# sijieaaa/AGPlace

Measured on AMD Instinct MI355X. Metric: aerial-ground pairs/sec (backbone+ODE+pool), higher is better.
Workload: dtype f16 (fp16 x fp16, fp32 accumulate); 1 GPU; nuScenes-AG 6-cam (C3/C4): MM.forward_q on [b,3,224,1344] + DBVanilla2D on [b,1,3,224,224], ResNet18 stem+layer1-3, euler h=0.1 x3 FCODE, GeM, stage-2 fusion; inference forward; the voxel branch's pooled outputs enter as fixed tensors (SURVEY.md 8d); global_batch=64, parallelism=dp1, bn=per-rank (eval: running statistics), paired_trunks=True, hipgraph=True, steps_in_flight=2, library_default_precision=4, headline_is_library_default=True, streams=2, query_sub_batches_on_streams=1, query_input=fp32 normalised panorama

## Files before the change

### agplace_amd/csrc/fblock64.hip

```cpp

#include <type_traits>
#include <utility>

#include "igemm_params.hpp"

namespace agp_fb {

constexpr int MAXP = 4;
constexpr int TW = 28;
constexpr int RING = 16;
constexpr int ROWB = 32 * 128;
constexpr int TAB_OFF = 2 * RING * ROWB + 512;
constexpr int STRIP_OFF = TAB_OFF + 4 * 64 * 4;
template <bool POOL> constexpr int lds_bytes() { return STRIP_OFF + 4 * 2048; }

struct Problem {
    const void* x; void* out;
    const void* w1; const void* w2;
    const float *s1, *t1, *s2, *t2;
    float* pool;
    uint32_t bytes;
    int VR, HP, W, pitch;
    int nstrips, segs;
    int dbg;
    FastDiv d_hp, d_segs;
};
struct Group {
    Problem p[MAXP];
    int wg_end[MAXP];
    int nprob;
};

__device__ __forceinline__ int perm23(int r) { return (r & 0x13) | ((r & 4) << 1) | ((r & 8) >> 1); }

template <bool POOL, bool M16, class... RF>
__global__ void __launch_bounds__(512, 2) fblock64_kernel(Group g, RF... rf) {
#if defined(__HIP_DEVICE_COMPILE__)
    constexpr bool RG = sizeof...(RF) != 0;
    extern __shared__ __attribute__((aligned(16))) char smem[];
    char* const XR = smem;
    char* const IR = smem + RING * ROWB;
    float* const tab = (float*)(smem + TAB_OFF);

    const int tid = threadIdx.x, lane = tid & 63;
    const int wave = __builtin_amdgcn_readfirstlane(tid >> 6);
    const int role = wave >> 2, cA = wave & 1, pA = (wave >> 1) & 1;
    const int l31 = lane & 31, lh = lane >> 5;
    const int la = lane & 15, kq = lane >> 4;

    const int bid = blockIdx.x;
    int pid = 0, lb = bid;
    {
        const int e0 = g.wg_end[0], e1 = g.wg_end[1], e2 = g.wg_end[2], np = g.nprob;
        if (np > 1 && bid >= e0) { pid = 1; lb = bid - e0; }
        if (np > 2 && bid >= e1) { pid = 2; lb = bid - e1; }
        if (np > 3 && bid >= e2) { pid = 3; lb = bid - e2; }
    }
    const Problem& p = g.p[pid];
    const int VR = p.VR, HP = p.HP, W = p.W, pitch = p.pitch, segs = p.segs;
    const FastDiv d_hp = p.d_hp;
    const int dbg = p.dbg;
    const int strip = (int)fdiv((uint32_t)lb, p.d_segs);
    const int sk = lb - strip * segs;
    const int Ra = (int)(((uint32_t)sk * (uint32_t)VR / (uint32_t)segs) & ~1u);
    const int Rb = sk + 1 == segs ? VR : (int)(((uint32_t)(sk + 1) * (uint32_t)VR / (uint32_t)segs) & ~1u);
    const int x0 = strip * TW;
    const int NS = (Rb - Ra + 3) >> 2;

    f16x8 w[36];
    {
        const bf16_t* wb = (const bf16_t*)(role ? p.w2 : p.w1);
        int i = 0;
        if constexpr (!M16) {
            const bf16_t* wp = wb + (size_t)(cA * 32 + perm23(l31)) * 576 + lh * 8;
#pragma unroll
            for (int ky = 0; ky < 3; ++ky)
#pragma unroll
                for (int cc = 0; cc < 2; ++cc)
#pragma unroll
                    for (int kx = 0; kx < 3; ++kx)
#pragma unroll
                        for (int ks = 0; ks < 2; ++ks, ++i)
                            w[i] = *(const f16x8*)(wp + (ky * 3 + kx) * 64 + cc * 32 + ks * 16);
        } else {
#pragma unroll
            for (int ky = 0; ky < 3; ++ky)
#pragma unroll
                for (int cc = 0; cc < 2; ++cc)
#pragma unroll
                    for (int kx = 0; kx < 3; ++kx)
#pragma unroll
                        for (int ct = 0; ct < 2; ++ct, ++i)
                            w[i] = *(const f16x8*)(wb + (size_t)(cA * 32 + 8 * (la >> 2) + 4 * ct + (la & 3)) * 576 + (ky * 3 + kx) * 64 + cc * 32 + kq * 8);
        }
    }
    if (tid < 64) {
        tab[tid] = p.s1[tid];
        tab[64 + tid] = p.t1[tid];
        tab[128 + tid] = p.s2[tid];
        tab[192 + tid] = p.t2[tid];
    }

    int A[3];
#pragma unroll
    for (int kx = 0; kx < 3; ++kx) {
        const int s = (M16 ? la : l31) + kx;
        A[kx] = s * 128 + (((M16 ? kq : lh) ^ ((s >> 1) & 7)) << 4);
    }
    const int px0 = M16 ? la : l31, px1 = M16 ? la + 16 : l31;
    const int ch0 = M16 ? kq : lh, ch1 = M16 ? kq : lh + 2;
    auto slot_off = [&](int s, int c) { return s * 128 + (((4 * cA + c) ^ ((s >> 1) & 7)) << 4); };
    const int wr0 = slot_off(px0, ch0), wr1 = slot_off(px1, ch1);
    const int rr0 = slot_off(px0 + 2, ch0), rr1 = slot_off(px1 + 2, ch1);
    const float* const tb0 = tab + role * 128 + 32 * cA + 8 * ch0;
    const float* const tb1 = tab + role * 128 + 32 * cA + 8 * ch1;
    const bool cin0 = (x0 - 1 + px0 >= 0) && (x0 - 1 + px0 < W), cin1 = (x0 - 1 + px1 >= 0) && (x0 - 1 + px1 < W);
    const bool ctk0 = cin0 && px0 < TW + 2, ctk1 = cin1 && px1 < TW + 2;
    const bool sok0 = px0 < TW && x0 + px0 < W, sok1 = px1 < TW && x0 + px1 < W;
    char* const ostrip = smem + STRIP_OFF + (wave & 3) * 2048;
    auto strip_off = [&](int px, int c) { return px * 64 + ((c ^ ((px >> 1) & 3)) << 4); };
    const int sw0 = strip_off(px0, ch0), sw1 = strip_off(px1, ch1);
    const int spx = lane >> 2;
    const int sr_ = strip_off(spx, lane & 3);
    const int gline = (x0 + 1 + spx) * 128 + 64 * cA + 16 * (lane & 3);
    const bool st_ok0 = spx < TW && x0 + spx < W, st_ok1 = spx + 16 < TW && x0 + spx + 16 < W;

    const __amdgpu_buffer_rsrc_t rx = __builtin_amdgcn_make_buffer_rsrc((void*)p.x, 0, p.bytes, 0x00020000);
    const int pc = wave & 3;
    int dvoff;
    {
        const int s = pc * 8 + (lane >> 3);
        int xp = x0 - 1 + s;
        xp = xp < 0 ? 0 : (xp > W + 1 ? W + 1 : xp);
        dvoff = xp * 128 + (((lane & 7) ^ ((s >> 1) & 7)) << 4);
    }
    auto issue_rows = [&](int R0, int cnt) {
#pragma unroll 4
        for (int r = 0; r < cnt; ++r) {
            const int R = R0 + r;
            const int Rc = R < 0 ? 0 : (R >= VR ? VR - 1 : R);
            const int so = __builtin_amdgcn_readfirstlane(Rc * pitch);
            __builtin_amdgcn_raw_ptr_buffer_load_lds(rx, LDS_PTR(XR + (R & (RING - 1)) * ROWB + pc * 1024), 16, dvoff, so, 0, 0);
        }
    };
    auto is_real = [&](int R) -> bool {
        if (R < 0 || R >= VR) return false;
        const int yy = R - (int)fdiv((uint32_t)R, d_hp) * HP;
        return yy >= 1 && yy <= HP - 2;
    };
    struct Acc {
        f32x16 m;
        f32x4 t[2][2];
    };
    auto acc_zero = [](Acc& a) {
        if constexpr (!M16) {
#pragma unroll
            for (int r = 0; r < 16; ++r) a.m[r] = 0.f;
        } else {
#pragma unroll
            for (int i = 0; i < 2; ++i)
#pragma unroll
                for (int j = 0; j < 2; ++j) a.t[i][j] = f32x4{0.f, 0.f, 0.f, 0.f};
        }
    };
    auto tile2 = [&](const char* ring, int R, Acc& a0, Acc& a1, auto&& mid, auto&& epi0) {
        acc_zero(a0);
        acc_zero(a1);
        constexpr int NG = M16 ? 24 : 48, PD = 2, NF = M16 ? 2 : 1;
        const char* rb[4];
#pragma unroll
        for (int q = 0; q < 4; ++q) rb[q] = ring + __builtin_amdgcn_readfirstlane(((R - 1 + q) & (RING - 1)) * ROWB);
        f16x8 fb[PD + 1][NF];
        auto load_group = [&](auto gc, auto slotc) {
            constexpr int g = decltype(gc)::value, sl = decltype(slotc)::value;
            if constexpr (M16) {
                constexpr int q = g / 6, cc = (g % 6) / 3, kx = g % 3;
                fb[sl][0] = *(const f16x8*)(rb[q] + (A[kx] ^ (cc << 6)));
                fb[sl][1] = *(const f16x8*)(rb[q] + (A[kx] ^ (cc << 6)) + 2048);
            } else {
                constexpr int q = g / 12, cc = (g % 12) / 6, kx = (g % 6) / 2, ks = g % 2;
                fb[sl][0] = *(const f16x8*)(rb[q] + (A[kx] ^ ((cc * 4 + ks * 2) << 4)));
            }
        };
        auto do_group = [&](auto gc, auto slotc) {
            constexpr int g = decltype(gc)::value, sl = decltype(slotc)::value;
            if constexpr (M16) {
                constexpr int q = g / 6, j = (g % 6) * 2;
#pragma unroll
                for (int ct = 0; ct < 2; ++ct) {
                    if constexpr (q <= 2) {
                        a0.t[ct][0] = __builtin_amdgcn_mfma_f32_16x16x32_f16(w[q * 12 + j + ct], fb[sl][0], a0.t[ct][0], 0, 0, 0);
                        a0.t[ct][1] = __builtin_amdgcn_mfma_f32_16x16x32_f16(w[q * 12 + j + ct], fb[sl][1], a0.t[ct][1], 0, 0, 0);
                    }
                    if constexpr (q >= 1) {
                        a1.t[ct][0] = __builtin_amdgcn_mfma_f32_16x16x32_f16(w[(q - 1) * 12 + j + ct], fb[sl][0], a1.t[ct][0], 0, 0, 0);
                        a1.t[ct][1] = __builtin_amdgcn_mfma_f32_16x16x32_f16(w[(q - 1) * 12 + j + ct], fb[sl][1], a1.t[ct][1], 0, 0, 0);
                    }
                }
            } else {
                constexpr int q = g / 12, j = g % 12;
                if constexpr (q <= 2) a0.m = __builtin_amdgcn_mfma_f32_32x32x16_f16(w[q * 12 + j], fb[sl][0], a0.m, 0, 0, 0);
                if constexpr (q >= 1) a1.m = __builtin_amdgcn_mfma_f32_32x32x16_f16(w[(q - 1) * 12 + j], fb[sl][0], a1.m, 0, 0, 0);
            }
        };
        auto step = [&](auto gc, auto&& self) -> void {
            constexpr int g = decltype(gc)::value;
            if constexpr (g < NG) {
                if constexpr (g + PD < NG) load_group(std::integral_constant<int, g + PD>{}, std::integral_constant<int, (g + PD) % (PD + 1)>{});
                __builtin_amdgcn_sched_barrier(0);
                do_group(gc, std::integral_constant<int, g % (PD + 1)>{});
                __builtin_amdgcn_sched_barrier(0);
                if constexpr (g == (M16 ? 4 : 8)) mid();
                if constexpr (g == 3 * NG / 4 - 1) epi0();
                self(std::integral_constant<int, g + 1>{}, self);
            }
        };
        load_group(std::integral_constant<int, 0>{}, std::integral_constant<int, 0>{});
        load_group(std::integral_constant<int, 1>{}, std::integral_constant<int, 1>{});
        if constexpr (PD > 2) load_group(std::integral_constant<int, 2>{}, std::integral_constant<int, 2>{});
        step(std::integral_constant<int, 0>{}, step);
    };
    auto bn = [&](const Acc& a, float* v) {
#pragma unroll
        for (int u = 0; u < 2; ++u) {
            const float* tb = u ? tb1 : tb0;
            const f32x4 s0 = *(const f32x4*)(tb), s1 = *(const f32x4*)(tb + 4);
            const f32x4 t0 = *(const f32x4*)(tb + 64), t1 = *(const f32x4*)(tb + 64 + 4);
#pragma unroll
            for (int e = 0; e < 4; ++e) {
                const float c0 = M16 ? a.t[0][u][e] : a.m[8 * u + e], c1 = M16 ? a.t[1][u][e] : a.m[8 * u + 4 + e];
                v[8 * u + e] = c0 * s0[e] + t0[e];
                v[8 * u + 4 + e] = c1 * s1[e] + t1[e];
            }
        }
    };
    RangeTrack<RG> rg;
    auto track16 = [&](const float* v, bool ok0, bool ok1) {
        RangeTrack<RG> t0, t1;
#pragma unroll
        for (int e = 0; e < 8; e += 2) { t0.pos2(v[e], v[e + 1]); t1.pos2(v[8 + e], v[9 + e]); }
        rg.pos2(ok0 ? t0.hi : 0.f, ok1 ? t1.hi : 0.f);
    };
    auto write_ir = [&](int R, const Acc& acc, bool real) {
        char* const dst = IR + __builtin_amdgcn_readfirstlane((R & (RING - 1)) * ROWB);
        float v[16];
        bn(acc, v);
        if constexpr (RG) track16(v, real && ctk0, real && ctk1);
        u32x4 o0 = pack8_h_lo(v, 0.f), o1 = pack8_h_lo(v + 8, 0.f);
        if (!(real && cin0)) o0 = u32x4{0u, 0u, 0u, 0u};
        if (!(real && cin1)) o1 = u32x4{0u, 0u, 0u, 0u};
        *(u32x4*)(dst + wr0) = o0;
        *(u32x4*)(dst + wr1) = o1;
    };
    auto conv1_pair = [&](int R) {
        const bool real0 = is_real(R), real1 = is_real(R + 1);
        Acc a0, a1;
        if (real0 || real1) {
            tile2(XR, R, a0, a1, [] {}, [&] { write_ir(R, a0, real0); });
            write_ir(R + 1, a1, real1);
        } else {
            acc_zero(a0);
            write_ir(R, a0, false);
            write_ir(R + 1, a0, false);
        }
    };
    f32x4 pacc[2];
    const __amdgpu_buffer_rsrc_t ro = __builtin_amdgcn_make_buffer_rsrc(p.out, 0, p.bytes, 0x00020000);
    u32x4 pl0 = {0u, 0u, 0u, 0u}, pl1 = {0u, 0u, 0u, 0u};
    int poff = -1;
    const int gl0 = st_ok0 ? gline : -(1 << 30), gl1 = st_ok1 ? gline + 2048 : -(1 << 30);
    auto store_lines = [&](const u32x4& l0, const u32x4& l1, int off) {
        const int v0 = (off >= 0 && gl0 >= 0) ? off + gl0 : -16, v1 = (off >= 0 && gl1 >= 0) ? off + gl1 : -16;
        if (!(dbg & 1)) {
            __builtin_amdgcn_raw_buffer_store_b128(l0, ro, v0, 0, 0);
            __builtin_amdgcn_raw_buffer_store_b128(l1, ro, v1, 0, 0);
        }
    };
    auto flush_pending = [&]() { store_lines(pl0, pl1, poff); poff = -1; };
    auto epi2 = [&](int R, const Acc& acc, bool real, u32x4& l0, u32x4& l1, bool first) {
        const char* const rsrc = XR + __builtin_amdgcn_readfirstlane((R & (RING - 1)) * ROWB);
        u32x4 r0 = {0u, 0u, 0u, 0u}, r1 = r0;
        if (!(dbg & 16)) { r0 = *(const u32x4*)(rsrc + rr0); r1 = *(const u32x4*)(rsrc + rr1); }
        float v[16], rf[16];
        bn(acc, v);
        unpack8_h(r0, rf);
        unpack8_h(r1, rf + 8);
#pragma unroll
        for (int e = 0; e < 16; ++e) v[e] += rf[e];
        if constexpr (RG) track16(v, real && sok0, real && sok1);
        u32x4 o0 = pack8_h_lo(v, 0.f), o1 = pack8_h_lo(v + 8, 0.f);
        if constexpr (POOL) {
            if (!sok0) o0 = u32x4{0u, 0u, 0u, 0u};
            if (!sok1) o1 = u32x4{0u, 0u, 0u, 0u};
        }
        *(u32x4*)(ostrip + sw0) = o0;
        *(u32x4*)(ostrip + sw1) = o1;
        l0 = *(const u32x4*)(ostrip + sr_);
        l1 = *(const u32x4*)(ostrip + sr_ + 1024);
        if constexpr (POOL) {
            if (first) { pacc[0] = f32x4{0.f, 0.f, 0.f, 0.f}; pacc[1] = pacc[0]; }
            {
                const int tpx = 8 * (lane >> 4) + ((lane >> 2) & 3), pp = lane & 3;
                const int tr0 = tpx * 64 + (((pp >> 1) ^ ((tpx >> 1) & 3)) << 4) + 8 * (pp & 1);
                typedef __attribute__((ext_vector_type(4))) short s16x4;
                const uint32_t one2 = real ? 0x3C003C00u : 0u;
                const f16x8 ones = __builtin_bit_cast(f16x8, u32x4{one2, one2, one2, one2});
#pragma unroll
                for (int ct = 0; ct < 2; ++ct) {
                    const s16x4 b0 = __builtin_amdgcn_ds_read_tr16_b64_v4i16((__attribute__((address_space(3))) s16x4*)(ostrip + (tr0 ^ (32 * ct))));
                    const s16x4 b1 = __builtin_amdgcn_ds_read_tr16_b64_v4i16((__attribute__((address_space(3))) s16x4*)(ostrip + (((tr0 + 256) ^ 32) ^ (32 * ct))));
                    const bf16x8 bf = __builtin_shufflevector(b0, b1, 0, 1, 2, 3, 4, 5, 6, 7);
                    pacc[ct] = __builtin_amdgcn_mfma_f32_16x16x32_f16(ones, __builtin_bit_cast(f16x8, bf), pacc[ct], 0, 0, 0);
                }
            }
        }
    };
    auto conv2_pair = [&](int R) {
        const bool real0 = is_real(R), real1 = is_real(R + 1);
        if (!(real0 || real1)) {
            if constexpr (POOL) { pacc[0] = f32x4{0.f, 0.f, 0.f, 0.f}; pacc[1] = pacc[0]; }
            return;
        }
        Acc a0, a1;
        u32x4 q0, q1;
        tile2(IR, R, a0, a1, flush_pending, [&] { epi2(R, a0, real0, q0, q1, true); });
        epi2(R + 1, a1, real1, pl0, pl1, false);
        store_lines(q0, q1, real0 ? __builtin_amdgcn_readfirstlane(R * pitch) : -1);
        poff = real1 ? __builtin_amdgcn_readfirstlane((R + 1) * pitch) : -1;
    };
    auto pool_flush = [&](int R) {
        if constexpr (POOL) {
            if (p.pool != nullptr && lane < 16) {
                float* o = p.pool + ((size_t)(R >> 1) * p.nstrips + strip) * 64 + 32 * cA + lane;
                o[0] = pacc[0][0];
                o[16] = pacc[1][0];
            }
        }
    };

    if (role == 0) issue_rows(Ra - 2, 8);
    __builtin_amdgcn_s_waitcnt(0x0070);
    __builtin_amdgcn_s_barrier();
    if (role == 0 && pA == 0) conv1_pair(Ra - 1);
    asm volatile("s_waitcnt lgkmcnt(0)" ::: "memory");
    __builtin_amdgcn_s_barrier();
    for (int t = 0; t <= NS; ++t) {
        if (role == 0) {
            if (t < NS) {
                if (t + 1 < NS && !(dbg & 2)) issue_rows(Ra + 4 * t + 6, 4);
                const int R = Ra + 1 + 4 * t + 2 * pA;
                if (R <= Rb) conv1_pair(R);
            }
            asm volatile("s_waitcnt vmcnt(0)" ::: "memory");
        } else if (t >= 1) {
            const int R = Ra + 4 * (t - 1) + 2 * pA;
            if (R < Rb) {
                conv2_pair(R);
                pool_flush(R);
            }
        }
        asm volatile("s_waitcnt lgkmcnt(0)" ::: "memory");
        if (!(dbg & 4)) __builtin_amdgcn_s_barrier();
    }
    if (role == 1) flush_pending();
    rg.flush(rg_word(rf...), 0.f);
#endif
}

}

using namespace agp_fb;

static int fb_num_cus() {
    static int n = -1;
    if (n < 0) {
        int dev = 0, v = 0;
        if (hipGetDevice(&dev) != hipSuccess || hipDeviceGetAttribute(&v, hipDeviceAttributeMultiprocessorCount, dev) != hipSuccess || v <= 0) v = 256;
        n = v;
    }
    return n;
}

static bool fb_desc_ok(const agp_bblock64_desc* d) {
    return d && d->in && d->out && d->w1 && d->w2 && d->scale1 && d->shift1 && d->scale2 && d->shift2 && d->n > 0 && d->h > 0 && d->w > 0 &&
           (d->h & 1) == 0 && (int64_t)d->n * (d->h + 2) * (d->w + 2) * 128 < (1ll << 31);
}

extern "C" int64_t agp_bblock64_pool_floats(const agp_bblock64_desc* d) {
    if (!fb_desc_ok(d)) return 0;
    return (int64_t)d->n * ((d->h + 2) / 2) * ((d->w + TW - 1) / TW) * 64;
}

extern "C" int agp_bblock64_fwd_grouped(const agp_bblock64_desc* descs, int n, void* stream) {
    if (!descs || n < 1 || n > MAXP) return AGP_E_BADARG;
    Group g = {};
    g.nprob = n;
    bool pool = false;
    int64_t total = 0;
    for (int i = 0; i < n; ++i) {
        const agp_bblock64_desc* d = descs + i;
        if (!fb_desc_ok(d)) return AGP_E_BADARG;
        Problem& p = g.p[i];
        p.x = d->in; p.out = d->out; p.w1 = d->w1; p.w2 = d->w2;
        p.s1 = d->scale1; p.t1 = d->shift1; p.s2 = d->scale2; p.t2 = d->shift2;
        p.pool = d->pool_partial;
        pool = pool || d->pool_partial;
        p.HP = d->h + 2; p.VR = d->n * p.HP; p.W = d->w; p.pitch = (d->w + 2) * 128;
        p.bytes = (uint32_t)((int64_t)p.VR * p.pitch);
        p.nstrips = (d->w + TW - 1) / TW;
        p.d_hp = make_fastdiv((uint32_t)p.HP);
        p.dbg = AGP_TUNE("FB_DBG", 0);
        total += (int64_t)p.nstrips * p.VR;
    }
    const int cus = fb_num_cus();
    int wg = 0;
    for (int i = 0; i < n; ++i) {
        Problem& p = g.p[i];
        int64_t s = (int64_t)p.VR * cus / total;
        const int64_t smax = p.VR / 16 > 1 ? p.VR / 16 : 1;
        s = s < 1 ? 1 : (s > smax ? smax : s);
        while (s > 1 && s * (int64_t)p.VR >= (1ll << 32)) --s;
        p.segs = (int)s;
        p.d_segs = make_fastdiv((uint32_t)p.segs);
        wg += p.nstrips * p.segs;
        g.wg_end[i] = wg;
    }
    const int form = descs[0].form == 0 ? 1 : 0;
    static std::atomic<uint64_t> attr_done[2][2][2];
    uint32_t* const rflag = agp_range_flag_get();
    auto launch = [&](auto... rf) {
        constexpr bool RG = sizeof...(rf) != 0;
        const void* fn = pool ? (form ? (const void*)fblock64_kernel<true, true, decltype(rf)...> : (const void*)fblock64_kernel<true, false, decltype(rf)...>)
                              : (form ? (const void*)fblock64_kernel<false, true, decltype(rf)...> : (const void*)fblock64_kernel<false, false, decltype(rf)...>);
        const int lds = pool ? lds_bytes<true>() : lds_bytes<false>();
        if (!agp_lds_attr(fn, lds, attr_done[RG][pool][form])) return AGP_E_LAUNCH;
        (void)hipGetLastError();
        if (pool && form) hipLaunchKernelGGL((fblock64_kernel<true, true, decltype(rf)...>), dim3(wg), dim3(512), lds, (hipStream_t)stream, g, rf...);
        else if (pool) hipLaunchKernelGGL((fblock64_kernel<true, false, decltype(rf)...>), dim3(wg), dim3(512), lds, (hipStream_t)stream, g, rf...);
        else if (form) hipLaunchKernelGGL((fblock64_kernel<false, true, decltype(rf)...>), dim3(wg), dim3(512), lds, (hipStream_t)stream, g, rf...);
        else hipLaunchKernelGGL((fblock64_kernel<false, false, decltype(rf)...>), dim3(wg), dim3(512), lds, (hipStream_t)stream, g, rf...);
        AGP_CHECK_LAUNCH();
        return AGP_OK;
    };
    return rflag ? launch(rflag) : launch();
}

__global__ void __launch_bounds__(1024) bblock64_pool_finish_kernel(const float* __restrict__ partial, int cnt, float inv_hw,
                                                                    float* __restrict__ mean_out) {
    __shared__ float red[16][64];
    const int im = blockIdx.x, c = threadIdx.x & 63, k = threadIdx.x >> 6;
    const float* base = partial + (size_t)im * cnt * 64 + c;
    float s = 0.f;
    for (int b0 = k; b0 < cnt; b0 += 16 * 8) {
        float v[8];
#pragma unroll
        for (int u = 0; u < 8; ++u) {
            const int b = b0 + 16 * u;
            v[u] = b < cnt ? base[(size_t)b * 64] : 0.f;
        }
#pragma unroll
        for (int u = 0; u < 8; ++u) s += v[u];
    }
    red[k][c] = s;
    __syncthreads();
    if (k == 0) {
        float t[8];
#pragma unroll
        for (int u = 0; u < 8; ++u) t[u] = red[2 * u][c] + red[2 * u + 1][c];
        mean_out[(size_t)im * 64 + c] = (((t[0] + t[1]) + (t[2] + t[3])) + ((t[4] + t[5]) + (t[6] + t[7]))) * inv_hw;
    }
}

extern "C" int agp_bblock64_pool_finish(const float* partial, int n, int h, int w, float* mean_out, void* stream) {
    if (!partial || !mean_out || n <= 0 || h <= 0 || w <= 0 || (h & 1)) return AGP_E_BADARG;
    AGP_LAUNCH(bblock64_pool_finish_kernel, dim3(n), dim3(1024), 0, (hipStream_t)stream, partial, (h + 2) / 2 * ((w + TW - 1) / TW),
               1.f / ((float)h * (float)w), mean_out);
    AGP_CHECK_LAUNCH();
    return AGP_OK;
}
```

Before: 41780 pairs/s.

## Iterate fused basic block over real row pairs, skipping padding rows

The fused ResNet basic-block kernel now walks over real output row pairs instead of padded virtual rows. Image top and bottom borders are served from a shared zeroed LDS row rather than from computed padding rows, which removes the per-row is_real checks and the wasted conv work on halo rows. Segment boundaries now fall on pairs and a seam flag decides when the halo pair has to be recomputed. The launcher also hands leftover CUs greedily to the problems with the heaviest load. The costs are extra index arithmetic (fastdiv per row), a more complex seam and pool-zero path, and a risk of boundary-correctness bugs.

```diff
diff --git a/agplace_amd/csrc/fblock64.hip b/agplace_amd/csrc/fblock64.hip
--- a/agplace_amd/csrc/fblock64.hip
+++ b/agplace_amd/csrc/fblock64.hip
@@ -12,7 +12,9 @@
 constexpr int ROWB = 32 * 128;
 constexpr int TAB_OFF = 2 * RING * ROWB + 512;
 constexpr int STRIP_OFF = TAB_OFF + 4 * 64 * 4;
-template <bool POOL> constexpr int lds_bytes() { return STRIP_OFF + 4 * 2048; }
+constexpr int ZROW_OFF = STRIP_OFF + 4 * 2048;
+constexpr int ZROW_BYTES = ROWB + 512;
+template <bool POOL> constexpr int lds_bytes() { return ZROW_OFF + ZROW_BYTES; }
 
 struct Problem {
     const void* x; void* out;
@@ -20,10 +22,10 @@
     const float *s1, *t1, *s2, *t2;
     float* pool;
     uint32_t bytes;
-    int VR, HP, W, pitch;
+    int VR, NP, J, W, pitch;
     int nstrips, segs;
     int dbg;
-    FastDiv d_hp, d_segs;
+    FastDiv d_j, d_segs;
 };
 struct Group {
     Problem p[MAXP];
@@ -57,15 +59,17 @@
         if (np > 3 && bid >= e2) { pid = 3; lb = bid - e2; }
     }
     const Problem& p = g.p[pid];
-    const int VR = p.VR, HP = p.HP, W = p.W, pitch = p.pitch, segs = p.segs;
-    const FastDiv d_hp = p.d_hp;
+    const int NP = p.NP, J = p.J, W = p.W, pitch = p.pitch, segs = p.segs;
+    const FastDiv d_j = p.d_j;
     const int dbg = p.dbg;
     const int strip = (int)fdiv((uint32_t)lb, p.d_segs);
     const int sk = lb - strip * segs;
-    const int Ra = (int)(((uint32_t)sk * (uint32_t)VR / (uint32_t)segs) & ~1u);
-    const int Rb = sk + 1 == segs ? VR : (int)(((uint32_t)(sk + 1) * (uint32_t)VR / (uint32_t)segs) & ~1u);
+    const int Pa = (int)((uint32_t)sk * (uint32_t)NP / (uint32_t)segs);
+    const int Pb = sk + 1 == segs ? NP : (int)((uint32_t)(sk + 1) * (uint32_t)NP / (uint32_t)segs);
     const int x0 = strip * TW;
-    const int NS = (Rb - Ra + 3) >> 2;
+    const int NS = (Pb - Pa + 1) >> 1;
+    const bool seam_a = Pa != (int)fdiv((uint32_t)Pa, d_j) * J;
+    const int Pe1 = Pb != (int)fdiv((uint32_t)Pb, d_j) * J ? Pb : Pb - 1;
 
     f16x8 w[36];
     {
@@ -100,6 +104,7 @@
         tab[128 + tid] = p.s2[tid];
         tab[192 + tid] = p.t2[tid];
     }
+    if (tid < ZROW_BYTES / 16) *(u32x4*)(smem + ZROW_OFF + tid * 16) = u32x4{0u, 0u, 0u, 0u};
 
     int A[3];
 #pragma unroll
@@ -134,19 +139,27 @@
         xp = xp < 0 ? 0 : (xp > W + 1 ? W + 1 : xp);
         dvoff = xp * 128 + (((lane & 7) ^ ((s >> 1) & 7)) << 4);
     }
-    auto issue_rows = [&](int R0, int cnt) {
-#pragma unroll 4
+    auto vrow = [&](int c) { return c + 2 * (int)fdiv((uint32_t)(c >> 1), d_j) + 1; };
+    auto issue_rows = [&](int c0, int cnt) {
+#pragma unroll 2
         for (int r = 0; r < cnt; ++r) {
-            const int R = R0 + r;
-            const int Rc = R < 0 ? 0 : (R >= VR ? VR - 1 : R);
-            const int so = __builtin_amdgcn_readfirstlane(Rc * pitch);
-            __builtin_amdgcn_raw_ptr_buffer_load_lds(rx, LDS_PTR(XR + (R & (RING - 1)) * ROWB + pc * 1024), 16, dvoff, so, 0, 0);
-        }
-    };
-    auto is_real = [&](int R) -> bool {
-        if (R < 0 || R >= VR) return false;
-        const int yy = R - (int)fdiv((uint32_t)R, d_hp) * HP;
-        return yy >= 1 && yy <= HP - 2;
+            const int c = c0 + r;
+            const int cc = c < 0 ? 0 : (c >= 2 * NP ? 2 * NP - 1 : c);
+            const int so = __builtin_amdgcn_readfirstlane(vrow(cc) * pitch);
+            __builtin_amdgcn_raw_ptr_buffer_load_lds(rx, LDS_PTR(XR + (c & (RING - 1)) * ROWB + pc * 1024), 16, dvoff, so, 0, 0);
+        }
+    };
+    struct Pair {
+        int img, j;
+        bool top, bot;
+    };
+    auto pair_of = [&](int P) {
+        Pair q;
+        q.img = (int)fdiv((uint32_t)P, d_j);
+        q.j = P - q.img * J;
+        q.top = q.j == 0;
+        q.bot = q.j == J - 1;
+        return q;
     };
     struct Acc {
         f32x16 m;
@@ -163,13 +176,16 @@
                 for (int j = 0; j < 2; ++j) a.t[i][j] = f32x4{0.f, 0.f, 0.f, 0.f};
         }
     };
-    auto tile2 = [&](const char* ring, int R, Acc& a0, Acc& a1, auto&& mid, auto&& epi0) {
+    auto tile2 = [&](int ring, int c0, bool top, bool bot, Acc& a0, Acc& a1, auto&& mid, auto&& epi0) {
         acc_zero(a0);
         acc_zero(a1);
         constexpr int NG = M16 ? 24 : 48, PD = 2, NF = M16 ? 2 : 1;
         const char* rb[4];
 #pragma unroll
-        for (int q = 0; q < 4; ++q) rb[q] = ring + __builtin_amdgcn_readfirstlane(((R - 1 + q) & (RING - 1)) * ROWB);
+        for (int q = 0; q < 4; ++q) {
+            const bool z = (q == 0 && top) || (q == 3 && bot);
+            rb[q] = smem + __builtin_amdgcn_readfirstlane(z ? ZROW_OFF : ring + ((c0 - 1 + q) & (RING - 1)) * ROWB);
+        }
         f16x8 fb[PD + 1][NF];
         auto load_group = [&](auto gc, auto slotc) {
             constexpr int g = decltype(gc)::value, sl = decltype(slotc)::value;
@@ -241,28 +257,22 @@
         for (int e = 0; e < 8; e += 2) { t0.pos2(v[e], v[e + 1]); t1.pos2(v[8 + e], v[9 + e]); }
         rg.pos2(ok0 ? t0.hi : 0.f, ok1 ? t1.hi : 0.f);
     };
-    auto write_ir = [&](int R, const Acc& acc, bool real) {
-        char* const dst = IR + __builtin_amdgcn_readfirstlane((R & (RING - 1)) * ROWB);
+    auto write_ir = [&](int c, const Acc& acc) {
+        char* const dst = IR + __builtin_amdgcn_readfirstlane((c & (RING - 1)) * ROWB);
         float v[16];
         bn(acc, v);
-        if constexpr (RG) track16(v, real && ctk0, real && ctk1);
+        if constexpr (RG) track16(v, ctk0, ctk1);
         u32x4 o0 = pack8_h_lo(v, 0.f), o1 = pack8_h_lo(v + 8, 0.f);
-        if (!(real && cin0)) o0 = u32x4{0u, 0u, 0u, 0u};
-        if (!(real && cin1)) o1 = u32x4{0u, 0u, 0u, 0u};
+        if (!cin0) o0 = u32x4{0u, 0u, 0u, 0u};
+        if (!cin1) o1 = u32x4{0u, 0u, 0u, 0u};
         *(u32x4*)(dst + wr0) = o0;
         *(u32x4*)(dst + wr1) = o1;
     };
-    auto conv1_pair = [&](int R) {
-        const bool real0 = is_real(R), real1 = is_real(R + 1);
+    auto conv1_pair = [&](int P) {
+        const Pair q = pair_of(P);
         Acc a0, a1;
-        if (real0 || real1) {
-            tile2(XR, R, a0, a1, [] {}, [&] { write_ir(R, a0, real0); });
-            write_ir(R + 1, a1, real1);
-        } else {
-            acc_zero(a0);
-            write_ir(R, a0, false);
-            write_ir(R + 1, a0, false);
-        }
+        tile2(0, 2 * P, q.top, q.bot, a0, a1, [] {}, [&] { write_ir(2 * P, a0); });
+        write_ir(2 * P + 1, a1);
     };
     f32x4 pacc[2];
     const __amdgpu_buffer_rsrc_t ro = __builtin_amdgcn_make_buffer_rsrc(p.out, 0, p.bytes, 0x00020000);
@@ -277,8 +287,8 @@
         }
     };
     auto flush_pending = [&]() { store_lines(pl0, pl1, poff); poff = -1; };
-    auto epi2 = [&](int R, const Acc& acc, bool real, u32x4& l0, u32x4& l1, bool first) {
-        const char* const rsrc = XR + __builtin_amdgcn_readfirstlane((R & (RING - 1)) * ROWB);
+    auto epi2 = [&](int c, const Acc& acc, u32x4& l0, u32x4& l1, bool first) {
+        const char* const rsrc = XR + __builtin_amdgcn_readfirstlane((c & (RING - 1)) * ROWB);
         u32x4 r0 = {0u, 0u, 0u, 0u}, r1 = r0;
         if (!(dbg & 16)) { r0 = *(const u32x4*)(rsrc + rr0); r1 = *(const u32x4*)(rsrc + rr1); }
         float v[16], rf[16];
@@ -287,7 +297,7 @@
         unpack8_h(r1, rf + 8);
 #pragma unroll
         for (int e = 0; e < 16; ++e) v[e] += rf[e];
-        if constexpr (RG) track16(v, real && sok0, real && sok1);
+        if constexpr (RG) track16(v, sok0, sok1);
         u32x4 o0 = pack8_h_lo(v, 0.f), o1 = pack8_h_lo(v + 8, 0.f);
         if constexpr (POOL) {
             if (!sok0) o0 = u32x4{0u, 0u, 0u, 0u};
@@ -303,7 +313,7 @@
                 const int tpx = 8 * (lane >> 4) + ((lane >> 2) & 3), pp = lane & 3;
                 const int tr0 = tpx * 64 + (((pp >> 1) ^ ((tpx >> 1) & 3)) << 4) + 8 * (pp & 1);
                 typedef __attribute__((ext_vector_type(4))) short s16x4;
-                const uint32_t one2 = real ? 0x3C003C00u : 0u;
+                const uint32_t one2 = 0x3C003C00u;
                 const f16x8 ones = __builtin_bit_cast(f16x8, u32x4{one2, one2, one2, one2});
 #pragma unroll
                 for (int ct = 0; ct < 2; ++ct) {
@@ -315,49 +325,43 @@
             }
         }
     };
-    auto conv2_pair = [&](int R) {
-        const bool real0 = is_real(R), real1 = is_real(R + 1);
-        if (!(real0 || real1)) {
-            if constexpr (POOL) { pacc[0] = f32x4{0.f, 0.f, 0.f, 0.f}; pacc[1] = pacc[0]; }
-            return;
-        }
+    auto conv2_pair = [&](int P) {
+        const Pair q = pair_of(P);
+        const int V = 2 * P + 2 * q.img + 1;
         Acc a0, a1;
         u32x4 q0, q1;
-        tile2(IR, R, a0, a1, flush_pending, [&] { epi2(R, a0, real0, q0, q1, true); });
-        epi2(R + 1, a1, real1, pl0, pl1, false);
-        store_lines(q0, q1, real0 ? __builtin_amdgcn_readfirstlane(R * pitch) : -1);
-        poff = real1 ? __builtin_amdgcn_readfirstlane((R + 1) * pitch) : -1;
-    };
-    auto pool_flush = [&](int R) {
+        tile2(RING * ROWB, 2 * P, q.top, q.bot, a0, a1, flush_pending, [&] { epi2(2 * P, a0, q0, q1, true); });
+        epi2(2 * P + 1, a1, pl0, pl1, false);
+        store_lines(q0, q1, __builtin_amdgcn_readfirstlane(V * pitch));
+        poff = __builtin_amdgcn_readfirstlane((V + 1) * pitch);
         if constexpr (POOL) {
             if (p.pool != nullptr && lane < 16) {
-                float* o = p.pool + ((size_t)(R >> 1) * p.nstrips + strip) * 64 + 32 * cA + lane;
+                const int es = p.nstrips * 64;
+                float* o = p.pool + (size_t)(q.img * (J + 1) + q.j) * es + strip * 64 + 32 * cA + lane;
                 o[0] = pacc[0][0];
                 o[16] = pacc[1][0];
-            }
-        }
-    };
-
-    if (role == 0) issue_rows(Ra - 2, 8);
+                if (q.bot) { o[es] = 0.f; o[es + 16] = 0.f; }
+            }
+        }
+    };
+
+    if (role == 0) issue_rows(2 * Pa - 3, 10);
     __builtin_amdgcn_s_waitcnt(0x0070);
     __builtin_amdgcn_s_barrier();
-    if (role == 0 && pA == 0) conv1_pair(Ra - 1);
+    if (role == 0 && (pA == 1 || seam_a)) conv1_pair(Pa - 1 + pA);
     asm volatile("s_waitcnt lgkmcnt(0)" ::: "memory");
     __builtin_amdgcn_s_barrier();
     for (int t = 0; t <= NS; ++t) {
         if (role == 0) {
             if (t < NS) {
-                if (t + 1 < NS && !(dbg & 2)) issue_rows(Ra + 4 * t + 6, 4);
-                const int R = Ra + 1 + 4 * t + 2 * pA;
-                if (R <= Rb) conv1_pair(R);
+                if (t + 1 < NS && !(dbg & 2)) issue_rows(2 * Pa + 4 * t + 7, 4);
+                const int P = Pa + 2 * t + 1 + pA;
+                if (P <= Pe1) conv1_pair(P);
             }
             asm volatile("s_waitcnt vmcnt(0)" ::: "memory");
         } else if (t >= 1) {
-            const int R = Ra + 4 * (t - 1) + 2 * pA;
-            if (R < Rb) {
-                conv2_pair(R);
-                pool_flush(R);
-            }
+            const int P = Pa + 2 * (t - 1) + pA;
+            if (P < Pb) conv2_pair(P);
         }
         asm volatile("s_waitcnt lgkmcnt(0)" ::: "memory");
         if (!(dbg & 4)) __builtin_amdgcn_s_barrier();
@@ -405,22 +409,42 @@
         p.s1 = d->scale1; p.t1 = d->shift1; p.s2 = d->scale2; p.t2 = d->shift2;
         p.pool = d->pool_partial;
         pool = pool || d->pool_partial;
-        p.HP = d->h + 2; p.VR = d->n * p.HP; p.W = d->w; p.pitch = (d->w + 2) * 128;
+        p.J = d->h / 2; p.NP = d->n * p.J; p.VR = d->n * (d->h + 2); p.W = d->w; p.pitch = (d->w + 2) * 128;
         p.bytes = (uint32_t)((int64_t)p.VR * p.pitch);
         p.nstrips = (d->w + TW - 1) / TW;
-        p.d_hp = make_fastdiv((uint32_t)p.HP);
+        p.d_j = make_fastdiv((uint32_t)p.J);
         p.dbg = AGP_TUNE("FB_DBG", 0);
-        total += (int64_t)p.nstrips * p.VR;
+        total += (int64_t)p.nstrips * p.NP;
     }
     const int cus = fb_num_cus();
+    int64_t segs[MAXP], smax[MAXP];
+    int64_t rem = cus;
+    for (int i = 0; i < n; ++i) {
+        const Problem& p = g.p[i];
+        smax[i] = p.NP / 8 > 1 ? p.NP / 8 : 1;
+        while (smax[i] > 1 && smax[i] * (int64_t)p.VR >= (1ll << 32)) --smax[i];
+        const int64_t s = (int64_t)p.NP * cus / total;
+        segs[i] = s < 1 ? 1 : (s > smax[i] ? smax[i] : s);
+        rem -= p.nstrips * segs[i];
+    }
+    for (;;) {
+        int best = -1;
+        for (int i = 0; i < n; ++i) {
+            const Problem& p = g.p[i];
+            if (segs[i] >= smax[i] || p.nstrips > rem) continue;
+            if (best < 0) { best = i; continue; }
+            const Problem& b = g.p[best];
+            const int64_t li = (int64_t)p.NP * segs[best], lb = (int64_t)b.NP * segs[i];
+            if (li > lb || (li == lb && (int64_t)p.nstrips * p.NP > (int64_t)b.nstrips * b.NP)) best = i;
+        }
+        if (best < 0) break;
+        ++segs[best];
+        rem -= g.p[best].nstrips;
+    }
     int wg = 0;
     for (int i = 0; i < n; ++i) {
         Problem& p = g.p[i];
-        int64_t s = (int64_t)p.VR * cus / total;
-        const int64_t smax = p.VR / 16 > 1 ? p.VR / 16 : 1;
-        s = s < 1 ? 1 : (s > smax ? smax : s);
-        while (s > 1 && s * (int64_t)p.VR >= (1ll << 32)) --s;
-        p.segs = (int)s;
+        p.segs = (int)segs[i];
         p.d_segs = make_fastdiv((uint32_t)p.segs);
         wg += p.nstrips * p.segs;
         g.wg_end[i] = wg;
```

After: 42390 pairs/s (median of 6 runs). +1.5%, better.
